# jgsimard/big-dreamer

Measured on AMD Instinct MI355X. Metric: latent transitions/sec (RSSM + imagination) at batch=50 chunk=50 H=15, higher is better.
Workload: dtype f32

## Files before the change

### big_dreamer_amd/_cabi.py

```python
from __future__ import annotations

import ctypes as C
import os

import torch

_HERE = os.path.dirname(os.path.abspath(__file__))
LIB_PATH = os.environ.get("BD_LIB") or os.path.join(_HERE, "libbigdreamer_hip.so")

if not os.path.exists(LIB_PATH):
    raise ImportError(
        f"{LIB_PATH} is missing: the MI355X HIP extension has not been built "
        "(run `python -c 'import __graft_entry__ as g; g.build()'`). There is no CPU fallback.")

lib = C.CDLL(LIB_PATH)

BD_MAX_LAYERS = 6
ACT_NONE, ACT_ELU, ACT_ELU_GRAD = 0, 1, 2
ACT_RELU, ACT_RELU_GRAD, ACT_TANH, ACT_TANH_GRAD = 3, 4, 5, 6
CNN_ACTS = {"ELU": (ACT_ELU, ACT_ELU_GRAD), "ReLU": (ACT_RELU, ACT_RELU_GRAD), "Tanh": (ACT_TANH, ACT_TANH_GRAD)}
GRAD_ACTS = (ACT_ELU_GRAD, ACT_RELU_GRAD, ACT_TANH_GRAD)
P = C.c_void_p
F32 = C.c_float
I32 = C.c_int
# ... 245 lines not shown
    "bd_scan_lds_bytes": (C.c_size_t, [I32] * 8),
    "bd_observe_cluster_set_spin_limit": (I32, [C.c_uint]),
    "bd_observe_cluster_set_ksplit": (I32, [I32]),
    "bd_gauss_head_forward": (I32, [P, P, I32, I32, F32, P, P, P, P]),
    "bd_gauss_head_backward": (I32, [P, P, P, P, P, I32, I32, P, P]),
    "bd_observe_cat_forward": (I32, [C.POINTER(ObserveCatFwdArgs), P]),
    "bd_observe_cat_backward": (I32, [C.POINTER(ObserveCatBwdArgs), P]),
    "bd_observe_cat_cluster_size": (I32, [I32, I32, I32, I32, I32]),
    "bd_observe_cat_cluster_ws_floats": (C.c_size_t, [I32, I32, I32, I32, I32]),
    "bd_observe_cat_forward_cluster": (I32, [C.POINTER(ObserveCatFwdArgs), I32, P, C.c_size_t, P]),
    "bd_observe_cat_backward_cluster": (I32, [C.POINTER(ObserveCatBwdArgs), I32, P, C.c_size_t, P]),
    "bd_imagine_cat_forward": (I32, [C.POINTER(ImagineCatFwdArgs), P]),
    "bd_imagine_cat_backward": (I32, [C.POINTER(ImagineCatBwdArgs), P]),
    "bd_imagine_forward": (I32, [C.POINTER(ImagineFwdArgs), P]),
    "bd_imagine_forward_scan": (I32, [C.POINTER(ImagineFwdArgs), P]),
    "bd_actor_entropy": (I32, [P, P, P, I32, I32, I32, I32, P]),
    "bd_imagine_backward": (I32, [C.POINTER(ImagineBwdArgs), P]),
    "bd_lambda_return_forward": (I32, [P, P, I32, I32, F32, F32, P, P]),
    "bd_rng_fill": (I32, [C.POINTER(RngFillArgs), P]),
    "bd_philox4x32_10": (I32, [C.POINTER(C.c_uint), C.POINTER(C.c_uint), C.POINTER(C.c_uint)]),
    "bd_actor_entropy_rng": (I32, [C.c_ulonglong, C.c_ulonglong, C.c_uint, P, P, I32, I32, I32, I32, P]),
    "bd_gemm_nt": (I32, [P, I32, P, I32, P, I32, I32, I32, I32, I32, P]),
    "bd_categorical_head_forward": (I32, [P, P, I32, I32, I32, P, P, P]),
    "bd_categorical_head_backward": (I32, [P, P, I32, I32, I32, P, P]),
    "bd_kl_categorical_forward": (I32, [P, P, I32, I32, I32, F32, I32, P, I32, P, P]),
    "bd_kl_categorical_backward": (I32, [P, P, I32, I32, I32, F32, F32, F32, F32, P, I32, P, P, P]),
    "bd_plan_rollout": (I32, [C.POINTER(PlanArgs), P]),
    "bd_cem_refit": (I32, [P, I32, P, I32, I32, I32, I32, I32, P, P, P]),
    "bd_plan_rollout_cat": (I32, [C.POINTER(PlanCatArgs), P]),
    "bd_act_step_supported": (I32, [I32, I32, I32, I32, I32, I32]),
    "bd_act_step": (I32, [C.POINTER(ActArgs), P]),
    "bd_act_step_cat_supported": (I32, [I32] * 10),
    "bd_act_step_cat": (I32, [C.POINTER(ActCatArgs), P]),
    "bd_tanh_normal_mode": (I32, [P, P, P, C.c_ulonglong, C.c_ulonglong, C.c_uint, I32, I32, I32, P, P, P]),
    "bd_lambda_return_backward": (I32, [P, F32, I32, I32, F32, F32, P, P, P]),
    "bd_img_heads_supported": (I32, [I32, I32]),
    "bd_img_heads_fwd_bwd": (I32, [C.POINTER(ImgHeadsArgs), P]),
    "bd_actor_reinforce": (I32, [P, P, P, P, P, P, P, I32, I32, I32, F32, F32, F32, I32, P, P, I32, P, P]),
    "bd_actor_reinforce_cat": (I32, [P, P, P, P, P, P, I32, I32, I32, F32, F32, F32, I32, P, P, I32, P, P]),
    "bd_normal_nll": (I32, [P, I32, P, I32, I32, I32, F32, P, I32, P, I32, P, P]),
    "bd_bernoulli_nll": (I32, [P, P, C.c_size_t, F32, P, P, I32, P, P]),
    "bd_kl_forward": (I32, [P, P, P, P, I32, I32, F32, I32, P, I32, P, P]),
    "bd_kl_backward": (I32, [P, P, P, P, I32, I32, F32, F32, F32, F32, P, I32, P, P, P, P, P]),
    "bd_sum": (I32, [P, C.c_size_t, P, I32, P, P]),
    "bd_sumsq": (I32, [P, C.c_size_t, P, I32, P, P]),
    "bd_adam_step": (I32, [P, P, P, P, C.c_size_t, F32, F32, F32, F32, F32, I32, F32, P, I32, P]),
    "bd_polyak": (I32, [P, P, C.c_size_t, F32, P]),
    "bd_replay_gather": (I32, [P, P, I32, I32, P, P]),
    "bd_replay_gather_pixels": (I32, [P, P, I32, I32, I32, P, P, P]),
    "bd_replay_gather_pixels_rng": (I32, [P, P, I32, I32, I32, C.c_ulonglong, C.c_ulonglong, P, P]),
    "bd_replay_append": (I32, [C.POINTER(ReplayAppendArgs), P]),
    "bd_replay_sample_gather": (I32, [C.POINTER(ReplaySampleArgs), P]),
    "bd_reduce_ws_floats": (C.c_size_t, []),
    "bd_conv_gemm": (I32, [C.POINTER(ConvArgs), P]),
    "bd_conv_thin_forward": (I32, [P, I32, I32, I32, I32, I32, P, I32, P, I32, P, P, P]),
    "bd_conv_pack_class": (I32, [P, P, I32, I32, I32, I32, I32, I32, I32, P]),
    "bd_conv_pack_fused": (I32, [P, P, I32, I32, I32, P]),
    "bd_act_backward": (I32, [P, P, C.c_size_t, I32, P]),
    "bd_elu_backward": (I32, [P, P, C.c_size_t, P]),
    "bd_image_layout": (I32, [P, P, I32, I32, I32, I32, P]),
    "bd_eval_frame": (I32, [P, P, I32, U8P, I32, I32, P]),
    "bd_openl_video": (I32, [P, P, I32, I32, U8P, P]),
    "bd_openl_error": (I32, [P, P, I32, I32, I32, I32, P, P]),
    "bd_colsum_ws_floats": (C.c_size_t, [I32]),
    "bd_colsum": (I32, [P, C.c_size_t, I32, P, P, P]),
    "bd_fingerprint": (I32, [C.POINTER(FingerprintArgs), P, P]),
    "bd_diag_ws_floats": (C.c_size_t, []),
    "bd_moments": (I32, [C.POINTER(MomentsArgs), P, P, P]),
    "bd_latent_stats": (I32, [P, P, P, P, I32, I32, P, P, P, P]),
    "bd_latent_stats_categorical": (I32, [P, P, I32, I32, I32, P, P, P, P, P]),
    "bd_segment_sumsq": (I32, [P, I32, C.POINTER(C.c_size_t), P, P, P]),
    "bd_return_range": (I32, [P, I32, I32, I32, C.c_double, C.c_double, P, P, P]),
    "bd_return_seed": (I32, [P, F32, P, C.c_size_t, P, P, I32, P]),
    "bd_actor_reinforce_norm": (I32, [P, P, P, P, P, P, P, P, I32, I32, I32, F32, F32, F32, I32, P, P, I32, P, P]),
    "bd_actor_reinforce_cat_norm": (I32, [P, P, P, P, P, P, P, I32, I32, I32, F32, F32, F32, I32, P, P, I32, P, P]),
    "bd_twohot_decode": (I32, [P, I32, I32, I32, F32, P, P, P]),
    "bd_twohot_decode_backward": (I32, [P, I32, P, I32, I32, F32, P, I32, P]),
    "bd_twohot_nll": (I32, [P, I32, P, P, I32, I32, F32, F32, P, I32, P, P, P]),
}

for _name, (_res, _args) in _SIGS.items():
    _fn = getattr(lib, _name)
    _fn.restype = _res
    _fn.argtypes = _args

EXPORTED = tuple(_SIGS)


def check(rc: int) -> None:
    if rc != 0:
        raise RuntimeError("bigdreamer_hip: " + lib.bd_last_error().decode())


def ptr(t) -> int:
    if t is None:
        return None
    if not (t.dtype in (torch.float32, torch.int64, torch.uint8) and t.is_cuda):
        raise TypeError("expected a CUDA fp32/int64/uint8 tensor")
    if not (t.is_contiguous() or (t.dim() == 2 and t.stride(1) == 1 and t.stride(0) >= t.shape[1])):
        raise ValueError(f"non-contiguous tensor (shape {tuple(t.shape)}, strides {t.stride()}) passed to a HIP kernel: "
                         "call .contiguous() first")
    return t.data_ptr()


def stream() -> int:
    return torch.cuda.current_stream().cuda_stream
# ... 5 lines not shown
```

### big_dreamer_amd/csrc/reduce.hip

```cpp
#include "bd_device.h"
#include "bd_host.h"
#include "bd_discrete.h"
#include "bd_latent.h"

namespace bd {

constexpr int kRedBlocks = 1024;
constexpr float kHalfLog2Pi = 0.91893853320467274178f;

static inline int red_blocks(size_t n) {
    size_t b = (n + 255) / 256;
    return (int)(b < 1 ? 1 : (b > kRedBlocks ? kRedBlocks : b));
}

__global__ __launch_bounds__(256) void final_sum_kernel(const double* __restrict__ partials, int n,
                                                        float* __restrict__ scalars, int slot) {
    __shared__ double red[kWaves];
    double s = 0.0;
    for (int i = threadIdx.x; i < n; i += blockDim.x) s += partials[i];
    s = block_sum_d(s, red);
    if (threadIdx.x == 0) scalars[slot] = (float)s;
}

template <int MODE>
__global__ __launch_bounds__(256) void sum_kernel(const float* __restrict__ x, size_t n, double* __restrict__ partials) {
    __shared__ double red[kWaves];
    double s = 0.0;
    for (size_t i = (size_t)blockIdx.x * blockDim.x + threadIdx.x; i < n; i += (size_t)gridDim.x * blockDim.x) {
        const float v = x[i];
        s += MODE ? (double)v * v : (double)v;
    }
    s = block_sum_d(s, red);
    if (threadIdx.x == 0) partials[blockIdx.x] = s;
}

__global__ __launch_bounds__(256) void normal_nll_kernel(const float* __restrict__ pred, int ldp,
                                                         const float* __restrict__ target, int ldt, int rows, int D,
                                                         float grad_scale, float* __restrict__ dpred, int ldd,
                                                         double* __restrict__ partials) {
    __shared__ double red[kWaves];
    double s = 0.0;
    const size_t n = (size_t)rows * D;
    for (size_t i = (size_t)blockIdx.x * blockDim.x + threadIdx.x; i < n; i += (size_t)gridDim.x * blockDim.x) {
        const size_t r = i / D, c = i - r * D;
        const float d = pred[r * ldp + c] - target[r * ldt + c];
        s += (double)(0.5f * d * d + kHalfLog2Pi);
        if (dpred) dpred[r * ldd + c] = d * grad_scale;
    }
    s = block_sum_d(s, red);
    if (threadIdx.x == 0) partials[blockIdx.x] = s;
}

__global__ __launch_bounds__(256) void bernoulli_nll_kernel(const float* __restrict__ logits, const float* __restrict__ target,
                                                            size_t n, float grad_scale, float* __restrict__ dlogits,
                                                            double* __restrict__ partials) {
    __shared__ double red[kWaves];
    double s = 0.0;
    for (size_t i = (size_t)blockIdx.x * blockDim.x + threadIdx.x; i < n; i += (size_t)gridDim.x * blockDim.x) {
        const float x = logits[i], t = target[i];
        s += (double)(fmaxf(x, 0.f) - x * t + log1pf(expf(-fabsf(x))));
        if (dlogits) dlogits[i] = (1.f / (1.f + expf(-x)) - t) * grad_scale;
    }
    s = block_sum_d(s, red);
    if (threadIdx.x == 0) partials[blockIdx.x] = s;
}

__global__ __launch_bounds__(256) void kl_fwd_kernel(const float* __restrict__ qm, const float* __restrict__ qs,
                                                     const float* __restrict__ pm, const float* __restrict__ ps,
                                                     int rows, int S, float free_nats, int sum_form,
                                                     double* __restrict__ partials) {
    __shared__ double red[kWaves];
    double s = 0.0;
    if (!sum_form) {
        const size_t n = (size_t)rows * S;
        for (size_t i = (size_t)blockIdx.x * blockDim.x + threadIdx.x; i < n; i += (size_t)gridDim.x * blockDim.x)
            s += (double)kl_elem(qm[i], qs[i], pm[i], ps[i]);
    } else {
        for (size_t r = (size_t)blockIdx.x * blockDim.x + threadIdx.x; r < (size_t)rows;
             r += (size_t)gridDim.x * blockDim.x) {
            float rs = 0.f;
            for (int c = 0; c < S; ++c) {
                const size_t i = r * S + c;
                rs += kl_elem(qm[i], qs[i], pm[i], ps[i]);
            }
            s += (double)fmaxf(rs, free_nats);
        }
    }
    s = block_sum_d(s, red);
    if (threadIdx.x == 0) partials[blockIdx.x] = s;
}

__device__ __forceinline__ float max_grad(float x, float fn) { return x < fn ? 0.f : (x == fn ? 0.5f : 1.f); }

__global__ __launch_bounds__(256) void kl_bwd_kernel(const float* __restrict__ qm, const float* __restrict__ qs,
                                                     const float* __restrict__ pm, const float* __restrict__ ps,
                                                     int rows, int S, float free_nats, float kl_balance, float weight,
                                                     float inv_count, const float* __restrict__ scalars, int slot,
                                                     float* __restrict__ dqm, float* __restrict__ dqs,
                                                     float* __restrict__ dpm, float* __restrict__ dps) {
    const size_t n = (size_t)rows * S;
    const bool sum_form = kl_balance == -1.f;
    float fq, fp;
    if (!sum_form) {
        const float f = max_grad(scalars[slot] * inv_count, free_nats) * weight * inv_count;
        fp = kl_balance * f;
        fq = (1.f - kl_balance) * f;
    } else {
        fq = fp = weight / (float)rows;
    }
    for (size_t i = (size_t)blockIdx.x * blockDim.x + threadIdx.x; i < n; i += (size_t)gridDim.x * blockDim.x) {
        float gq = fq, gp = fp;
        if (sum_form) {
            const size_t r = i / S;
            float rs = 0.f;
            for (int c = 0; c < S; ++c) {
                const size_t j = r * S + c;
                rs += kl_elem(qm[j], qs[j], pm[j], ps[j]);
            }
            const float f = max_grad(rs, free_nats);
            gq *= f;
            gp *= f;
        }
        const float a = qm[i], b = qs[i], c = pm[i], d = ps[i];
        const float inv_d = 1.f / d, inv_d2 = inv_d * inv_d, diff = a - c;
        dqm[i] = gq * diff * inv_d2;
        dqs[i] = gq * (b * inv_d2 - 1.f / b);
        dpm[i] = -gp * diff * inv_d2;
        dps[i] = gp * (inv_d - (b * b + diff * diff) * inv_d2 * inv_d);
    }
}

__global__ __launch_bounds__(256) void gauss_head_fwd_kernel(const float* __restrict__ out, const float* __restrict__ eps,
                                                             int M, int S, float min_std, float* __restrict__ mean,
                                                             float* __restrict__ std, float* __restrict__ state) {
    const size_t n = (size_t)M * S;
    for (size_t i = (size_t)blockIdx.x * blockDim.x + threadIdx.x; i < n; i += (size_t)gridDim.x * blockDim.x) {
        const size_t r = i / S, c = i - r * S;
        const float m = out[r * 2 * S + c];
        const float sd = softplusf(out[r * 2 * S + S + c]) + min_std;
        if (mean) mean[i] = m;
        if (std) std[i] = sd;
        if (state) state[i] = m + sd * eps[i];
// ... 5 lines not shown
                                                             const float* __restrict__ dmean,
                                                             const float* __restrict__ dstd, int M, int S,
                                                             float* __restrict__ dout) {
    const size_t n = (size_t)M * S;
    for (size_t i = (size_t)blockIdx.x * blockDim.x + threadIdx.x; i < n; i += (size_t)gridDim.x * blockDim.x) {
        const size_t r = i / S, c = i - r * S;
        const float ds = dstate ? dstate[i] : 0.f;
        const float gm = ds + (dmean ? dmean[i] : 0.f);
        const float gs = (dstate ? ds * eps[i] : 0.f) + (dstd ? dstd[i] : 0.f);
        dout[r * 2 * S + c] = gm;
        dout[r * 2 * S + S + c] = gs * sigmoidf(out[r * 2 * S + S + c]);
    }
}

__global__ __launch_bounds__(256) void lambda_fwd_kernel(const float* __restrict__ reward, const float* __restrict__ value,
                                                         int Hm, int N, float disc, float lam, float* __restrict__ ret) {
    const float one_minus = 1.f - lam, dl = disc * lam;
    for (int n = blockIdx.x * blockDim.x + threadIdx.x; n < N; n += gridDim.x * blockDim.x) {
        const float boot = value[(size_t)(Hm - 1) * N + n];
        float last = boot;
        for (int t = Hm - 1; t >= 0; --t) {
            const float next = (t == Hm - 1) ? boot : value[(size_t)(t + 1) * N + n];
            const float inp = reward[(size_t)t * N + n] + disc * next * one_minus;
            last = inp + dl * last;
            ret[(size_t)t * N + n] = last;
        }
    }
}

__global__ __launch_bounds__(256) void lambda_bwd_kernel(const float* __restrict__ dret, float dconst, int Hm, int N,
                                                         float disc, float lam, float* __restrict__ dreward,
                                                         float* __restrict__ dvalue) {
    const float c = disc * lam, w = disc * (1.f - lam);
    for (int n = blockIdx.x * blockDim.x + threadIdx.x; n < N; n += gridDim.x * blockDim.x) {
        float G = 0.f;
        for (int t = 0; t < Hm; ++t) {
            G = (dret ? dret[(size_t)t * N + n] : dconst) + c * G;
            dreward[(size_t)t * N + n] = G;
            if (t == 0 && Hm > 1) dvalue[n] = 0.f;
            if (t < Hm - 1) {
                dvalue[(size_t)(t + 1) * N + n] = G * w;
            } else {
                const float prev = (Hm > 1) ? dvalue[(size_t)t * N + n] : 0.f;
                dvalue[(size_t)t * N + n] = prev + G * w + c * G;
            }
        }
    }
}

__global__ __launch_bounds__(256) void actor_reinforce_kernel(
    const float* __restrict__ eps, const float* __restrict__ us, const float* __restrict__ stats,
    const float* __restrict__ ret, const float* __restrict__ base0, const float* __restrict__ value,
    const float* __restrict__ weight, const float* __restrict__ ret_scale, int rows, int N, int A, float scale,
    float dentropy, int write, float* __restrict__ dout, double* __restrict__ partials) {
    __shared__ double red[kWaves];
    constexpr float kLn2 = 0.69314718055994531f;
    if (ret_scale) scale /= ret_scale[0];
    double s = 0.0;
    for (int i = blockIdx.x * blockDim.x + threadIdx.x; i < rows; i += gridDim.x * blockDim.x) {
        const float w = weight ? weight[i] : 1.f;
        const float adv = ret[i] - (i < N ? base0[i] : value[i - N]);
        const float c = scale * w * adv;
        const float dent = dentropy * w;
        const float* e = eps + (size_t)i * A;
        const float* uu = us + (size_t)i * 2 * A;
        const float* st = stats + (size_t)i * 4 * A;
        float* d = dout + (size_t)i * 2 * A;
        float l = 0.f;
        for (int j = 0; j < A; ++j) {
            const float ej = e[j], u = uu[j], sd = uu[A + j];
            const float th = st[j], sg = st[A + j];
            const float x = -2.f * u;
            const float sp = fmaxf(x, 0.f) + log1pf(expf(-fabsf(x)));
            l += -0.5f * ej * ej - logf(sd) - kHalfLog2Pi - 2.f * (kLn2 - u - sp);
            const float inv = 1.f / sd, dth = 1.f - th * th;
            float gm = c * (ej * inv) * dth;
            float gr = c * ((ej * ej - 1.f) * inv) * sg;
            if (write) {
                gm += (dent * st[2 * A + j]) * dth;
                gr += (dent * st[3 * A + j]) * sg;
            } else {
                gm += d[j];
                gr += d[A + j];
            }
            d[j] = gm;
            d[A + j] = gr;
        }
        s += (double)(w * l * adv);
    }
    s = block_sum_d(s, red);
    if (threadIdx.x == 0) partials[blockIdx.x] = s;
}

__global__ __launch_bounds__(256) void actor_reinforce_cat_kernel(
    const float* __restrict__ action, const float* __restrict__ stats, const float* __restrict__ ret,
    const float* __restrict__ base0, const float* __restrict__ value, const float* __restrict__ weight,
    const float* __restrict__ ret_scale, int rows, int N, int A, float scale, float dentropy, int write,
    float* __restrict__ dout, double* __restrict__ partials) {
    __shared__ double red[kWaves];
    const int lane = threadIdx.x & 63;
    if (ret_scale) scale /= ret_scale[0];
    const int nw = gridDim.x * (blockDim.x >> 6);
    const bool valid = lane < A;
    double s = 0.0;
    for (int i = blockIdx.x * (blockDim.x >> 6) + (threadIdx.x >> 6); i < rows; i += nw) {
        const float w = weight ? weight[i] : 1.f;
        const float adv = ret[i] - (i < N ? base0[i] : value[i - N]);
        const float c = scale * w * adv;
        const size_t j = (size_t)i * A + lane;
        const float norm = valid ? stats[j] : -INFINITY;
        const unsigned long long hot = __ballot(valid && action[j] > 0.5f);
        const int k = hot ? __builtin_ctzll(hot) : 0;
        const float p = disc_probs(norm, valid);
        const float l = __shfl(norm, k, 64);
        float g = c * ((lane == k ? 1.f : 0.f) - p);
        if (write) {
            const float H = disc_entropy(norm, p, valid);
            g += (dentropy * w) * (-p * (norm + H));
        } else if (valid) {
            g += dout[j];
        }
        if (valid) dout[j] = g;
        if (lane == 0) s += (double)(w * l * adv);
    }
    s = block_sum_d(s, red);
    if (threadIdx.x == 0) partials[blockIdx.x] = s;
}

__global__ __launch_bounds__(256) void adam_kernel(float* __restrict__ p, float* __restrict__ g, float* __restrict__ m,
                                                   float* __restrict__ v, size_t n, float beta1, float beta2, float eps,
                                                   float wd, float step_size, float inv_sqrt_bc2, float max_norm,
                                                   const float* __restrict__ scalars, int sqnorm_slot) {
    const float total_norm = sqrtf(scalars[sqnorm_slot]);
    const float q = max_norm / (total_norm + 1e-6f);
    const float coef = q > 1.f ? 1.f : q;
    for (size_t i = (size_t)blockIdx.x * blockDim.x + threadIdx.x; i < n; i += (size_t)gridDim.x * blockDim.x) {
        const float gc = g[i] * coef;
        g[i] = gc;
        const float pi = p[i];
        const float gw = gc + wd * pi;
        const float mi = m[i] + (1.f - beta1) * (gw - m[i]);
        const float vi = v[i] * beta2 + (1.f - beta2) * gw * gw;
        m[i] = mi;
        v[i] = vi;
        const float denom = sqrtf(vi) * inv_sqrt_bc2 + eps;
        p[i] = pi - step_size * (mi / denom);
    }
}

__global__ __launch_bounds__(256) void polyak_kernel(float* __restrict__ t, const float* __restrict__ s, size_t n, float w) {
    for (size_t i = (size_t)blockIdx.x * blockDim.x + threadIdx.x; i < n; i += (size_t)gridDim.x * blockDim.x)
        t[i] = s[i] * w + t[i] * (1.f - w);
}

__global__ __launch_bounds__(256) void cat_head_fwd_kernel(const float* __restrict__ logits, const float* __restrict__ q,
                                                           size_t groups, int C, float* __restrict__ state,
                                                           float* __restrict__ probs) {
    const int l = threadIdx.x & 31;
    for (size_t g = (size_t)blockIdx.x * 8 + (threadIdx.x >> 5); g < groups; g += (size_t)gridDim.x * 8) {
        const size_t base = g * C;
        float lp[kCatPer];
        group_log_softmax(logits + base, C, l, lp);
        float pr[kCatPer], m = -INFINITY, s = 0.f;
#pragma unroll
        for (int i = 0; i < kCatPer; ++i) m = fmaxf(m, lp[i]);
        m = half_max(m);
#pragma unroll
        for (int i = 0; i < kCatPer; ++i) {
            pr[i] = (l + 32 * i < C) ? expf(lp[i] - m) : 0.f;
            s += pr[i];
        }
        s = half_sum(s);
        float best = -INFINITY;
        int arg = 0x7fffffff;
#pragma unroll
        for (int i = 0; i < kCatPer; ++i) {
            const int c = l + 32 * i;
            if (c < C) {
                pr[i] /= s;
                probs[base + c] = pr[i];
                const float r = pr[i] / q[base + c];
                if (r > best) { best = r; arg = c; }
            }
        }
#pragma unroll
        for (int o = 16; o > 0; o >>= 1) {
            const float ob = __shfl_xor(best, o, 64);
            const int oa = __shfl_xor(arg, o, 64);
            if (ob > best || (ob == best && oa < arg)) { best = ob; arg = oa; }
        }
#pragma unroll
        for (int i = 0; i < kCatPer; ++i) {
            const int c = l + 32 * i;
            if (c < C) state[base + c] = (c == arg) ? 1.f : 0.f;
        }
    }
}

__global__ __launch_bounds__(256) void cat_head_bwd_kernel(const float* __restrict__ dstate, const float* __restrict__ probs,
                                                           size_t groups, int C, float* __restrict__ dlogits) {
    const int l = threadIdx.x & 31;
    for (size_t g = (size_t)blockIdx.x * 8 + (threadIdx.x >> 5); g < groups; g += (size_t)gridDim.x * 8) {
        const size_t base = g * C;
        float pr[kCatPer], gr[kCatPer], dot = 0.f;
#pragma unroll
        for (int i = 0; i < kCatPer; ++i) {
            const int c = l + 32 * i;
            pr[i] = c < C ? probs[base + c] : 0.f;
            gr[i] = c < C ? dstate[base + c] : 0.f;
            dot += pr[i] * gr[i];
        }
        dot = half_sum(dot);
#pragma unroll
        for (int i = 0; i < kCatPer; ++i) {
            const int c = l + 32 * i;
            if (c < C) dlogits[base + c] = pr[i] * (gr[i] - dot);
        }
    }
}

__global__ __launch_bounds__(256) void cat_kl_fwd_kernel(const float* __restrict__ ql, const float* __restrict__ pl, int rows,
                                                         int D, int C, float free_nats, int sum_form,
                                                         double* __restrict__ partials) {
    __shared__ double red[kWaves > 4 ? kWaves : 4];
    const int l = threadIdx.x & 31;
    const size_t units = sum_form ? (size_t)rows : (size_t)rows * D;
    const int per = sum_form ? D : 1;
    double acc = 0.0;
    for (size_t u = (size_t)blockIdx.x * 8 + (threadIdx.x >> 5); u < units; u += (size_t)gridDim.x * 8) {
        float rs = 0.f;
        for (int d = 0; d < per; ++d) {
            const size_t base = (u * per + d) * C;
            float lq[kCatPer], lp[kCatPer];
            group_log_softmax(ql + base, C, l, lq);
            group_log_softmax(pl + base, C, l, lp);
            rs += group_kl(lq, lp, C, l);
        }
        if (l == 0) acc += (double)(sum_form ? fmaxf(rs, free_nats) : rs);
    }
    acc = block_sum_d(acc, red);
    if (threadIdx.x == 0) partials[blockIdx.x] = acc;
}

__global__ __launch_bounds__(256) void cat_kl_bwd_kernel(const float* __restrict__ ql, const float* __restrict__ pl, int rows,
                                                         int D, int C, float free_nats, float kl_balance, float weight,
                                                         float inv_count, const float* __restrict__ scalars, int slot,
                                                         float* __restrict__ dql, float* __restrict__ dpl) {
    const int l = threadIdx.x & 31;
    const bool sum_form = kl_balance == -1.f;
    const size_t units = sum_form ? (size_t)rows : (size_t)rows * D;
    const int per = sum_form ? D : 1;
    float fq, fp;
    if (!sum_form) {
        const float f = max_grad(scalars[slot] * inv_count, free_nats) * weight * inv_count;
        fp = kl_balance * f;
        fq = (1.f - kl_balance) * f;
    } else {
        fq = fp = weight / (float)rows;
    }
    for (size_t u = (size_t)blockIdx.x * 8 + (threadIdx.x >> 5); u < units; u += (size_t)gridDim.x * 8) {
        float f = 1.f;
        if (sum_form) {
            float rs = 0.f;
            for (int d = 0; d < per; ++d) {
                const size_t base = (u * per + d) * C;
                float lq[kCatPer], lp[kCatPer];
                group_log_softmax(ql + base, C, l, lq);
                group_log_softmax(pl + base, C, l, lp);
                rs += group_kl(lq, lp, C, l);
            }
            f = max_grad(rs, free_nats);
        }
        for (int d = 0; d < per; ++d) {
            const size_t base = (u * per + d) * C;
            float lq[kCatPer], lp[kCatPer];
            group_log_softmax(ql + base, C, l, lq);
            group_log_softmax(pl + base, C, l, lp);
            const float kl = group_kl(lq, lp, C, l);
#pragma unroll
            for (int i = 0; i < kCatPer; ++i) {
                const int c = l + 32 * i;
                if (c < C) {
                    const float qv = expf(lq[i]), pv = expf(lp[i]);
                    dql[base + c] = f * fq * (qv == 0.f ? 0.f : qv * (lq[i] - lp[i] - kl));
                    dpl[base + c] = f * fp * (pv - qv);
                }
            }
        }
    }
}

static int finish(double* partials, int nb, float* scalars, int slot, hipStream_t s, const char* name) {
    hipLaunchKernelGGL(final_sum_kernel, dim3(1), dim3(256), 0, s, partials, nb, scalars, slot);
    BD_CHECK_LAUNCH(name);
    return 0;
}

}

extern "C" {
using namespace bd;

size_t bd_reduce_ws_floats(void) { return 2 * (size_t)kRedBlocks; }

int bd_sum(const float* x, size_t n, float* scalars, int slot, float* ws, void* stream) {
    BD_REQUIRE(x && scalars && ws && n > 0, "bd_sum: bad arguments");
    const int nb = red_blocks(n);
    hipLaunchKernelGGL(sum_kernel<0>, dim3(nb), dim3(256), 0, (hipStream_t)stream, x, n, (double*)ws);
    BD_CHECK_LAUNCH("bd_sum");
    return finish((double*)ws, nb, scalars, slot, (hipStream_t)stream, "bd_sum(final)");
}

int bd_actor_reinforce_norm(const float* eps_action, const float* act_us, const float* act_stats, const float* returns,
                            const float* base0, const float* value, const float* weight, const float* ret_scale, int Hm,
                            int N, int A, float rho, float grad_scale, float dentropy, int write, float* d_actor_out,
                            float* scalars, int slot, float* ws, void* stream) {
    BD_REQUIRE(eps_action && act_us && act_stats && returns && base0 && (value || Hm == 1) && d_actor_out && scalars && ws,
               "bd_actor_reinforce: missing pointers");
    BD_REQUIRE(Hm > 0 && N > 0 && A > 0 && (size_t)Hm * N <= (size_t)INT32_MAX / 4 && slot >= 0,
               "bd_actor_reinforce: bad dims (Hm=%d N=%d A=%d slot=%d)", Hm, N, A, slot);
    BD_REQUIRE(rho >= 0.f && rho <= 1.f, "bd_actor_reinforce: gradient mixing %g outside [0, 1]", (double)rho);
    BD_REQUIRE(((size_t)ret_scale & 3u) == 0, "bd_actor_reinforce: ret_scale is not 4-byte aligned");
    const int rows = Hm * N;
    const int nb = red_blocks((size_t)rows);
    hipLaunchKernelGGL(actor_reinforce_kernel, dim3(nb), dim3(256), 0, (hipStream_t)stream, eps_action, act_us, act_stats,
                       returns, base0, value, weight, ret_scale, rows, N, A, -(1.f - rho) * grad_scale, dentropy, write,
                       d_actor_out, (double*)ws);
    BD_CHECK_LAUNCH("bd_actor_reinforce");
    return finish((double*)ws, nb, scalars, slot, (hipStream_t)stream, "bd_actor_reinforce(final)");
}

int bd_actor_reinforce(const float* eps_action, const float* act_us, const float* act_stats, const float* returns,
                       const float* base0, const float* value, const float* weight, int Hm, int N, int A, float rho,
                       float grad_scale, float dentropy, int write, float* d_actor_out, float* scalars, int slot, float* ws,
                       void* stream) {
    return bd_actor_reinforce_norm(eps_action, act_us, act_stats, returns, base0, value, weight, nullptr, Hm, N, A, rho,
                                   grad_scale, dentropy, write, d_actor_out, scalars, slot, ws, stream);
}

int bd_actor_reinforce_cat_norm(const float* action, const float* act_stats, const float* returns, const float* base0,
                                const float* value, const float* weight, const float* ret_scale, int Hm, int N, int A,
                                float rho, float grad_scale, float dentropy, int write, float* d_actor_out, float* scalars,
                                int slot, float* ws, void* stream) {
    BD_REQUIRE(action && act_stats && returns && base0 && (value || Hm == 1) && d_actor_out && scalars && ws,
               "bd_actor_reinforce_cat: missing pointers");
    BD_REQUIRE(Hm > 0 && N > 0 && A > 0 && A <= 64 && (size_t)Hm * N <= (size_t)INT32_MAX / 4 && slot >= 0,
               "bd_actor_reinforce_cat: bad dims (Hm=%d N=%d A=%d slot=%d)", Hm, N, A, slot);
    BD_REQUIRE(rho >= 0.f && rho <= 1.f, "bd_actor_reinforce_cat: gradient mixing %g outside [0, 1]", (double)rho);
    BD_REQUIRE(((size_t)ret_scale & 3u) == 0, "bd_actor_reinforce_cat: ret_scale is not 4-byte aligned");
    const int rows = Hm * N;
    const int nb = red_blocks((size_t)rows);
    hipLaunchKernelGGL(actor_reinforce_cat_kernel, dim3(nb), dim3(256), 0, (hipStream_t)stream, action, act_stats, returns,
                       base0, value, weight, ret_scale, rows, N, A, -(1.f - rho) * grad_scale, dentropy, write, d_actor_out,
                       (double*)ws);
    BD_CHECK_LAUNCH("bd_actor_reinforce_cat");
    return finish((double*)ws, nb, scalars, slot, (hipStream_t)stream, "bd_actor_reinforce_cat(final)");
}

int bd_actor_reinforce_cat(const float* action, const float* act_stats, const float* returns, const float* base0,
                           const float* value, const float* weight, int Hm, int N, int A, float rho, float grad_scale,
                           float dentropy, int write, float* d_actor_out, float* scalars, int slot, float* ws,
                           void* stream) {
    return bd_actor_reinforce_cat_norm(action, act_stats, returns, base0, value, weight, nullptr, Hm, N, A, rho, grad_scale,
                                       dentropy, write, d_actor_out, scalars, slot, ws, stream);
}

int bd_sumsq(const float* x, size_t n, float* scalars, int slot, float* ws, void* stream) {
    BD_REQUIRE(x && scalars && ws && n > 0, "bd_sumsq: bad arguments");
    const int nb = red_blocks(n);
    hipLaunchKernelGGL(sum_kernel<1>, dim3(nb), dim3(256), 0, (hipStream_t)stream, x, n, (double*)ws);
    BD_CHECK_LAUNCH("bd_sumsq");
    return finish((double*)ws, nb, scalars, slot, (hipStream_t)stream, "bd_sumsq(final)");
}

int bd_normal_nll(const float* pred, int ldp, const float* target, int ldt, int rows, int D, float grad_scale,
                  float* dpred, int ldd, float* scalars, int slot, float* ws, void* stream) {
    BD_REQUIRE(pred && target && scalars && ws && rows > 0 && D > 0, "bd_normal_nll: bad arguments");
    BD_REQUIRE(ldp >= D && ldt >= D && (!dpred || ldd >= D), "bd_normal_nll: leading dimension too small");
    const int nb = red_blocks((size_t)rows * D);
    hipLaunchKernelGGL(normal_nll_kernel, dim3(nb), dim3(256), 0, (hipStream_t)stream, pred, ldp, target, ldt, rows, D,
                       grad_scale, dpred, ldd, (double*)ws);
    BD_CHECK_LAUNCH("bd_normal_nll");
    return finish((double*)ws, nb, scalars, slot, (hipStream_t)stream, "bd_normal_nll(final)");
}

int bd_bernoulli_nll(const float* logits, const float* target, size_t n, float grad_scale, float* dlogits, float* scalars,
                     int slot, float* ws, void* stream) {
    BD_REQUIRE(logits && target && scalars && ws && n > 0, "bd_bernoulli_nll: bad arguments");
    const int nb = red_blocks(n);
    hipLaunchKernelGGL(bernoulli_nll_kernel, dim3(nb), dim3(256), 0, (hipStream_t)stream, logits, target, n, grad_scale,
                       dlogits, (double*)ws);
    BD_CHECK_LAUNCH("bd_bernoulli_nll");
    return finish((double*)ws, nb, scalars, slot, (hipStream_t)stream, "bd_bernoulli_nll(final)");
}

int bd_kl_forward(const float* qm, const float* qs, const float* pm, const float* ps, int rows, int S, float free_nats,
                  int sum_form, float* scalars, int slot, float* ws, void* stream) {
    BD_REQUIRE(qm && qs && pm && ps && scalars && ws && rows > 0 && S > 0, "bd_kl_forward: bad arguments");
    const int nb = red_blocks(sum_form ? (size_t)rows : (size_t)rows * S);
    hipLaunchKernelGGL(kl_fwd_kernel, dim3(nb), dim3(256), 0, (hipStream_t)stream, qm, qs, pm, ps, rows, S, free_nats,
                       sum_form, (double*)ws);
    BD_CHECK_LAUNCH("bd_kl_forward");
    return finish((double*)ws, nb, scalars, slot, (hipStream_t)stream, "bd_kl_forward(final)");
}

int bd_kl_backward(const float* qm, const float* qs, const float* pm, const float* ps, int rows, int S, float free_nats,
                   float kl_balance, float weight, float inv_count, const float* scalars, int slot, float* dqm,
                   float* dqs, float* dpm, float* dps, void* stream) {
    BD_REQUIRE(qm && qs && pm && ps && scalars && dqm && dqs && dpm && dps && rows > 0 && S > 0,
               "bd_kl_backward: bad arguments");
    hipLaunchKernelGGL(kl_bwd_kernel, dim3(red_blocks((size_t)rows * S)), dim3(256), 0, (hipStream_t)stream, qm, qs, pm,
                       ps, rows, S, free_nats, kl_balance, weight, inv_count, scalars, slot, dqm, dqs, dpm, dps);
    BD_CHECK_LAUNCH("bd_kl_backward");
    return 0;
}

int bd_gauss_head_forward(const float* out, const float* eps, int M, int S, float min_std, float* mean, float* std,
                          float* state, void* stream) {
    BD_REQUIRE(out && M > 0 && S > 0 && (!state || eps), "bd_gauss_head_forward: bad arguments");
    hipLaunchKernelGGL(gauss_head_fwd_kernel, dim3(red_blocks((size_t)M * S)), dim3(256), 0, (hipStream_t)stream, out, eps,
                       M, S, min_std, mean, std, state);
    BD_CHECK_LAUNCH("bd_gauss_head_forward");
    return 0;
}

int bd_gauss_head_backward(const float* out, const float* eps, const float* dstate, const float* dmean,
                           const float* dstd, int M, int S, float* dout, void* stream) {
    BD_REQUIRE(out && dout && M > 0 && S > 0 && (!dstate || eps), "bd_gauss_head_backward: bad arguments");
    hipLaunchKernelGGL(gauss_head_bwd_kernel, dim3(red_blocks((size_t)M * S)), dim3(256), 0, (hipStream_t)stream, out, eps,
                       dstate, dmean, dstd, M, S, dout);
    BD_CHECK_LAUNCH("bd_gauss_head_backward");
    return 0;
}

int bd_lambda_return_forward(const float* reward, const float* value, int Hm, int N, float discount, float lambda_,
                             float* returns, void* stream) {
    BD_REQUIRE(reward && value && returns && Hm > 0 && N > 0, "bd_lambda_return_forward: bad arguments");
    hipLaunchKernelGGL(lambda_fwd_kernel, dim3(red_blocks(N)), dim3(256), 0, (hipStream_t)stream, reward, value, Hm, N,
                       discount, lambda_, returns);
    BD_CHECK_LAUNCH("bd_lambda_return_forward");
    return 0;
}

int bd_lambda_return_backward(const float* dreturns, float dret_const, int Hm, int N, float discount, float lambda_,
                              float* dreward, float* dvalue, void* stream) {
    BD_REQUIRE(dreward && dvalue && Hm > 0 && N > 0, "bd_lambda_return_backward: bad arguments");
    hipLaunchKernelGGL(lambda_bwd_kernel, dim3(red_blocks(N)), dim3(256), 0, (hipStream_t)stream, dreturns, dret_const, Hm,
                       N, discount, lambda_, dreward, dvalue);
    BD_CHECK_LAUNCH("bd_lambda_return_backward");
    return 0;
}

int bd_adam_step(float* p, float* g, float* m, float* v, size_t n, float lr, float beta1, float beta2, float eps,
                 float weight_decay, int step, float max_norm, const float* scalars, int sqnorm_slot, void* stream) {
    BD_REQUIRE(p && g && m && v && scalars && n > 0 && step >= 1, "bd_adam_step: bad arguments");
    const double bc1 = 1.0 - pow((double)beta1, step), bc2 = 1.0 - pow((double)beta2, step);
    hipLaunchKernelGGL(adam_kernel, dim3(red_blocks(n)), dim3(256), 0, (hipStream_t)stream, p, g, m, v, n, beta1, beta2,
                       eps, weight_decay, (float)(lr / bc1), (float)(1.0 / sqrt(bc2)), max_norm, scalars, sqnorm_slot);
    BD_CHECK_LAUNCH("bd_adam_step");
    return 0;
}

int bd_polyak(float* target, const float* src, size_t n, float weight, void* stream) {
    BD_REQUIRE(target && src && n > 0, "bd_polyak: bad arguments");
    hipLaunchKernelGGL(polyak_kernel, dim3(red_blocks(n)), dim3(256), 0, (hipStream_t)stream, target, src, n, weight);
    BD_CHECK_LAUNCH("bd_polyak");
    return 0;
}

static inline int cat_blocks(size_t units) {
    size_t b = (units + 7) / 8;
    return (int)(b < 1 ? 1 : (b > (size_t)kRedBlocks ? (size_t)kRedBlocks : b));
}

int bd_categorical_head_forward(const float* logits, const float* q_noise, int rows, int D, int C, float* state,
                                float* probs, void* stream) {
    BD_REQUIRE(logits && q_noise && state && probs && rows > 0 && D > 0, "bd_categorical_head_forward: bad arguments");
    BD_REQUIRE(C > 0 && C <= 32 * kCatPer, "bd_categorical_head_forward: %d classes (max %d)", C, 32 * kCatPer);
    const size_t groups = (size_t)rows * D;
    hipLaunchKernelGGL(cat_head_fwd_kernel, dim3(cat_blocks(groups)), dim3(256), 0, (hipStream_t)stream, logits, q_noise,
                       groups, C, state, probs);
    BD_CHECK_LAUNCH("bd_categorical_head_forward");
    return 0;
}

int bd_categorical_head_backward(const float* dstate, const float* probs, int rows, int D, int C, float* dlogits,
                                 void* stream) {
    BD_REQUIRE(dstate && probs && dlogits && rows > 0 && D > 0, "bd_categorical_head_backward: bad arguments");
    BD_REQUIRE(C > 0 && C <= 32 * kCatPer, "bd_categorical_head_backward: %d classes (max %d)", C, 32 * kCatPer);
    const size_t groups = (size_t)rows * D;
    hipLaunchKernelGGL(cat_head_bwd_kernel, dim3(cat_blocks(groups)), dim3(256), 0, (hipStream_t)stream, dstate, probs,
                       groups, C, dlogits);
    BD_CHECK_LAUNCH("bd_categorical_head_backward");
    return 0;
}

int bd_kl_categorical_forward(const float* post_logits, const float* prior_logits, int rows, int D, int C, float free_nats,
                              int sum_form, float* scalars, int slot, float* ws, void* stream) {
    BD_REQUIRE(post_logits && prior_logits && scalars && ws && rows > 0 && D > 0, "bd_kl_categorical_forward: bad arguments");
    BD_REQUIRE(C > 0 && C <= 32 * kCatPer, "bd_kl_categorical_forward: %d classes (max %d)", C, 32 * kCatPer);
    const int nb = cat_blocks(sum_form ? (size_t)rows : (size_t)rows * D);
    hipLaunchKernelGGL(cat_kl_fwd_kernel, dim3(nb), dim3(256), 0, (hipStream_t)stream, post_logits, prior_logits, rows, D, C,
                       free_nats, sum_form, (double*)ws);
    BD_CHECK_LAUNCH("bd_kl_categorical_forward");
    return finish((double*)ws, nb, scalars, slot, (hipStream_t)stream, "bd_kl_categorical_forward(final)");
}

int bd_kl_categorical_backward(const float* post_logits, const float* prior_logits, int rows, int D, int C, float free_nats,
                               float kl_balance, float weight, float inv_count, const float* scalars, int slot,
                               float* dpost, float* dprior, void* stream) {
    BD_REQUIRE(post_logits && prior_logits && scalars && dpost && dprior && rows > 0 && D > 0,
               "bd_kl_categorical_backward: bad arguments");
    BD_REQUIRE(C > 0 && C <= 32 * kCatPer, "bd_kl_categorical_backward: %d classes (max %d)", C, 32 * kCatPer);
    const bool sum_form = kl_balance == -1.f;
    hipLaunchKernelGGL(cat_kl_bwd_kernel, dim3(cat_blocks(sum_form ? (size_t)rows : (size_t)rows * D)), dim3(256), 0,
                       (hipStream_t)stream, post_logits, prior_logits, rows, D, C, free_nats, kl_balance, weight, inv_count,
                       scalars, slot, dpost, dprior);
    BD_CHECK_LAUNCH("bd_kl_categorical_backward");
    return 0;
}

}
```

### include/bigdreamer_hip.h

```cpp
#ifndef BIGDREAMER_HIP_H
#define BIGDREAMER_HIP_H

#include <stddef.h>
#include <stdint.h>

#ifdef __cplusplus
extern "C" {
#endif

#define BD_MAX_LAYERS 6
#define BD_ACT_NONE 0
#define BD_ACT_ELU 1
#define BD_ACT_ELU_GRAD 2
#define BD_ACT_RELU 3
#define BD_ACT_RELU_GRAD 4
#define BD_ACT_TANH 5
#define BD_ACT_TANH_GRAD 6

const char* bd_last_error(void);
int bd_version(void);

#define BD_PACK_COPY 0
#define BD_PACK_PRODUCT 1
#define BD_PACK_PRODUCT_VEC 2
// ... 521 lines not shown
int bd_replay_gather(const float* src, const int64_t* idx, int n_idx, int width, float* dst, void* stream);

int bd_replay_gather_pixels(const unsigned char* src, const int64_t* idx, int n_idx, int pixels, int bit_depth,
                            const float* noise, float* dst, void* stream);
int bd_replay_gather_pixels_rng(const unsigned char* src, const int64_t* idx, int n_idx, int pixels, int bit_depth,
                                unsigned long long seed, unsigned long long step, float* dst, void* stream);

typedef struct {
    int n;
    int size;
    const int32_t* rows;
    const float* obs;
    int obs_width;
    int bit_depth;
    void* dst_obs;
    const float* act;
    int A;
    float* dst_act;
    const float* reward;
    const float* nonterminal;
    float* dst_reward;
    float* dst_nonterminal;
} bd_replay_append_args;
int bd_replay_append(const bd_replay_append_args* a, void* stream);

typedef struct {
    const void* obs;
    const float* act;
    const float* reward;
    const float* nonterminal;
    int obs_width;
    int A;
    int size;
    int lanes;
    int lane_size;
    int idx;
    int full;
    int n;
    int L;
    int bit_depth;
    unsigned long long seed;
    unsigned long long step;
    unsigned long long pix_seed;
    unsigned long long pix_step;
    float* dst_obs;
    float* dst_act;
    float* dst_reward;
    float* dst_nonterminal;
    int64_t* idx_out;
} bd_replay_sample_args;
int bd_replay_sample_gather(const bd_replay_sample_args* a, void* stream);

size_t bd_reduce_ws_floats(void);

#define BD_FP_MAX_BUFFERS 16
typedef struct {
    int n_buf;
    struct {
        const float* p;
        size_t n;
    } buf[BD_FP_MAX_BUFFERS];
} bd_fingerprint_args;
int bd_fingerprint(const bd_fingerprint_args* a, unsigned long long* out, void* stream);

size_t bd_diag_ws_floats(void);

#define BD_MOMENTS_MAX_BUFFERS 16
#define BD_MOMENTS_WORDS 6
typedef struct {
    int n_buf;
    struct {
        const float* p;
        const float* q;
        size_t n;
    } buf[BD_MOMENTS_MAX_BUFFERS];
} bd_moments_args;
int bd_moments(const bd_moments_args* a, double* out, float* ws, void* stream);

#define BD_LATENT_WORDS 15
int bd_latent_stats(const float* qm, const float* qs, const float* pm, const float* ps, int rows, int S, double* out,
                    double* colsum, float* ws, void* stream);

#define BD_LATENT_CAT_WORDS 5
int bd_latent_stats_categorical(const float* post_logits, const float* prior_logits, int rows, int D, int C, double* out,
                                double* colsum, unsigned* used, float* ws, void* stream);

#define BD_SEGMENTS_MAX 32
int bd_segment_sumsq(const float* x, int n_seg, const size_t* offsets, double* out, float* ws, void* stream);

int bd_return_range(const float* returns, int M, int k_lo, int k_hi, double decay, double floor_, double* state,
                    float* range, void* stream);
int bd_return_seed(const float* range, float dret_const, const float* weight, size_t n, float* dreturns, float* scalars,
                   int slot, void* stream);

int bd_twohot_decode(const float* logits, int ld, int rows, int K, float zmax, float* value, float* mean, void* stream);
int bd_twohot_decode_backward(const float* logits, int ld, const float* dvalue, int rows, int K, float zmax, float* dlogits,
                              int ldd, void* stream);
int bd_twohot_nll(const float* logits, int ld, const float* target, const float* weight, int rows, int K, float zmax,
                  float grad_scale, float* dlogits, int ldd, float* value, float* row_loss, void* stream);

#ifdef __cplusplus
}
#endif
#endif
```

Before: 13.99 million.

## Finish scalar reductions in-kernel via last-block atomic counter instead of second launch

```diff
diff --git a/big_dreamer_amd/_cabi.py b/big_dreamer_amd/_cabi.py
--- a/big_dreamer_amd/_cabi.py
+++ b/big_dreamer_amd/_cabi.py
@@ -321,6 +321,7 @@
     "bd_replay_append": (I32, [C.POINTER(ReplayAppendArgs), P]),
     "bd_replay_sample_gather": (I32, [C.POINTER(ReplaySampleArgs), P]),
     "bd_reduce_ws_floats": (C.c_size_t, []),
+    "bd_reduce_set_finish": (I32, [I32]),
     "bd_conv_gemm": (I32, [C.POINTER(ConvArgs), P]),
     "bd_conv_thin_forward": (I32, [P, I32, I32, I32, I32, I32, P, I32, P, I32, P, P, P]),
     "bd_conv_pack_class": (I32, [P, P, I32, I32, I32, I32, I32, I32, I32, P]),
diff --git a/big_dreamer_amd/csrc/reduce.hip b/big_dreamer_amd/csrc/reduce.hip
--- a/big_dreamer_amd/csrc/reduce.hip
+++ b/big_dreamer_amd/csrc/reduce.hip
@@ -1,9 +1,73 @@
+#include <atomic>
+#include <mutex>
+
 #include "bd_device.h"
 #include "bd_host.h"
 #include "bd_discrete.h"
 #include "bd_latent.h"
 
 namespace bd {
+
+constexpr int kFinishSets = 64;
+constexpr int kFinishShards = 32;
+constexpr int kFinishFlat = 64;
+static_assert(kFinishShards <= kFinishFlat, "the top word of a sharded grid counts kFinishShards arrivals");
+struct alignas(128) FinishWord {
+    unsigned v;
+    unsigned pad[31];
+};
+__device__ FinishWord finish_words[kFinishSets][1 + kFinishShards];
+
+struct Finish {
+    int set;
+    int slot;
+    float* scalars;
+};
+
+typedef __attribute__((address_space(1))) unsigned gu32;
+typedef __attribute__((address_space(1))) unsigned long long gu64;
+
+__device__ __forceinline__ void finish_block(double s, double* __restrict__ partials, const Finish& fin, double* red) {
+    const int nb = (int)gridDim.x, b = (int)blockIdx.x;
+    if (fin.set < 0) {
+        if (threadIdx.x == 0) partials[b] = s;
+        return;
+    }
+    __shared__ int last;
+    gu64* gp = (gu64*)(unsigned long long*)partials;
+    if (threadIdx.x == 0) {
+        __hip_atomic_store(gp + b, (unsigned long long)__double_as_longlong(s), __ATOMIC_RELAXED, __HIP_MEMORY_SCOPE_AGENT);
+        asm volatile("s_waitcnt vmcnt(0)" ::: "memory");
+        gu32* top = (gu32*)&finish_words[fin.set][0].v;
+        bool l;
+        if (nb <= kFinishFlat) {
+            l = __hip_atomic_fetch_add(top, 1u, __ATOMIC_RELAXED, __HIP_MEMORY_SCOPE_AGENT) == (unsigned)(nb - 1);
+        } else {
+            const int sh = b % kFinishShards;
+            const unsigned pop = (unsigned)((nb - sh + kFinishShards - 1) / kFinishShards);
+            gu32* sw = (gu32*)&finish_words[fin.set][1 + sh].v;
+            l = __hip_atomic_fetch_add(sw, 1u, __ATOMIC_RELAXED, __HIP_MEMORY_SCOPE_AGENT) == pop - 1;
+            if (l) {
+                __hip_atomic_store(sw, 0u, __ATOMIC_RELAXED, __HIP_MEMORY_SCOPE_AGENT);
+                l = __hip_atomic_fetch_add(top, 1u, __ATOMIC_RELAXED, __HIP_MEMORY_SCOPE_AGENT) ==
+                    (unsigned)(kFinishShards - 1);
+            }
+        }
+        if (l) {
+            __hip_atomic_store(top, 0u, __ATOMIC_RELAXED, __HIP_MEMORY_SCOPE_AGENT);
+            __builtin_amdgcn_fence(__ATOMIC_ACQUIRE, "agent");
+            asm volatile("s_waitcnt vmcnt(0)" ::: "memory");
+        }
+        last = l;
+    }
+    __syncthreads();
+    if (!last) return;
+    double t = 0.0;
+    for (int i = threadIdx.x; i < nb; i += blockDim.x)
+        t += __longlong_as_double((long long)__hip_atomic_load(gp + i, __ATOMIC_RELAXED, __HIP_MEMORY_SCOPE_AGENT));
+    t = block_sum_d(t, red);
+    if (threadIdx.x == 0) fin.scalars[fin.slot] = (float)t;
+}
 
 constexpr int kRedBlocks = 1024;
 constexpr float kHalfLog2Pi = 0.91893853320467274178f;
@@ -23,7 +87,7 @@
 }
 
 template <int MODE>
-__global__ __launch_bounds__(256) void sum_kernel(const float* __restrict__ x, size_t n, double* __restrict__ partials) {
+__global__ __launch_bounds__(256) void sum_kernel(const float* __restrict__ x, size_t n, double* __restrict__ partials, Finish fin) {
     __shared__ double red[kWaves];
     double s = 0.0;
     for (size_t i = (size_t)blockIdx.x * blockDim.x + threadIdx.x; i < n; i += (size_t)gridDim.x * blockDim.x) {
@@ -31,13 +95,13 @@
         s += MODE ? (double)v * v : (double)v;
     }
     s = block_sum_d(s, red);
-    if (threadIdx.x == 0) partials[blockIdx.x] = s;
+    finish_block(s, partials, fin, red);
 }
 
 __global__ __launch_bounds__(256) void normal_nll_kernel(const float* __restrict__ pred, int ldp,
                                                          const float* __restrict__ target, int ldt, int rows, int D,
                                                          float grad_scale, float* __restrict__ dpred, int ldd,
-                                                         double* __restrict__ partials) {
+                                                         double* __restrict__ partials, Finish fin) {
     __shared__ double red[kWaves];
     double s = 0.0;
     const size_t n = (size_t)rows * D;
@@ -48,12 +112,12 @@
         if (dpred) dpred[r * ldd + c] = d * grad_scale;
     }
     s = block_sum_d(s, red);
-    if (threadIdx.x == 0) partials[blockIdx.x] = s;
+    finish_block(s, partials, fin, red);
 }
 
 __global__ __launch_bounds__(256) void bernoulli_nll_kernel(const float* __restrict__ logits, const float* __restrict__ target,
                                                             size_t n, float grad_scale, float* __restrict__ dlogits,
-                                                            double* __restrict__ partials) {
+                                                            double* __restrict__ partials, Finish fin) {
     __shared__ double red[kWaves];
     double s = 0.0;
     for (size_t i = (size_t)blockIdx.x * blockDim.x + threadIdx.x; i < n; i += (size_t)gridDim.x * blockDim.x) {
@@ -62,13 +126,13 @@
         if (dlogits) dlogits[i] = (1.f / (1.f + expf(-x)) - t) * grad_scale;
     }
     s = block_sum_d(s, red);
-    if (threadIdx.x == 0) partials[blockIdx.x] = s;
+    finish_block(s, partials, fin, red);
 }
 
 __global__ __launch_bounds__(256) void kl_fwd_kernel(const float* __restrict__ qm, const float* __restrict__ qs,
                                                      const float* __restrict__ pm, const float* __restrict__ ps,
                                                      int rows, int S, float free_nats, int sum_form,
-                                                     double* __restrict__ partials) {
+                                                     double* __restrict__ partials, Finish fin) {
     __shared__ double red[kWaves];
     double s = 0.0;
     if (!sum_form) {
@@ -87,7 +151,7 @@
         }
     }
     s = block_sum_d(s, red);
-    if (threadIdx.x == 0) partials[blockIdx.x] = s;
+    finish_block(s, partials, fin, red);
 }
 
 __device__ __forceinline__ float max_grad(float x, float fn) { return x < fn ? 0.f : (x == fn ? 0.5f : 1.f); }
@@ -199,7 +263,7 @@
     const float* __restrict__ eps, const float* __restrict__ us, const float* __restrict__ stats,
     const float* __restrict__ ret, const float* __restrict__ base0, const float* __restrict__ value,
     const float* __restrict__ weight, const float* __restrict__ ret_scale, int rows, int N, int A, float scale,
-    float dentropy, int write, float* __restrict__ dout, double* __restrict__ partials) {
+    float dentropy, int write, float* __restrict__ dout, double* __restrict__ partials, Finish fin) {
     __shared__ double red[kWaves];
     constexpr float kLn2 = 0.69314718055994531f;
     if (ret_scale) scale /= ret_scale[0];
@@ -236,14 +300,14 @@
         s += (double)(w * l * adv);
     }
     s = block_sum_d(s, red);
-    if (threadIdx.x == 0) partials[blockIdx.x] = s;
+    finish_block(s, partials, fin, red);
 }
 
 __global__ __launch_bounds__(256) void actor_reinforce_cat_kernel(
     const float* __restrict__ action, const float* __restrict__ stats, const float* __restrict__ ret,
     const float* __restrict__ base0, const float* __restrict__ value, const float* __restrict__ weight,
     const float* __restrict__ ret_scale, int rows, int N, int A, float scale, float dentropy, int write,
-    float* __restrict__ dout, double* __restrict__ partials) {
+    float* __restrict__ dout, double* __restrict__ partials, Finish fin) {
     __shared__ double red[kWaves];
     const int lane = threadIdx.x & 63;
     if (ret_scale) scale /= ret_scale[0];
@@ -271,7 +335,7 @@
         if (lane == 0) s += (double)(w * l * adv);
     }
     s = block_sum_d(s, red);
-    if (threadIdx.x == 0) partials[blockIdx.x] = s;
+    finish_block(s, partials, fin, red);
 }
 
 __global__ __launch_bounds__(256) void adam_kernel(float* __restrict__ p, float* __restrict__ g, float* __restrict__ m,
@@ -368,7 +432,7 @@
 
 __global__ __launch_bounds__(256) void cat_kl_fwd_kernel(const float* __restrict__ ql, const float* __restrict__ pl, int rows,
                                                          int D, int C, float free_nats, int sum_form,
-                                                         double* __restrict__ partials) {
+                                                         double* __restrict__ partials, Finish fin) {
     __shared__ double red[kWaves > 4 ? kWaves : 4];
     const int l = threadIdx.x & 31;
     const size_t units = sum_form ? (size_t)rows : (size_t)rows * D;
@@ -386,7 +450,7 @@
         if (l == 0) acc += (double)(sum_form ? fmaxf(rs, free_nats) : rs);
     }
     acc = block_sum_d(acc, red);
-    if (threadIdx.x == 0) partials[blockIdx.x] = acc;
+    finish_block(acc, partials, fin, red);
 }
 
 __global__ __launch_bounds__(256) void cat_kl_bwd_kernel(const float* __restrict__ ql, const float* __restrict__ pl, int rows,
@@ -437,7 +501,25 @@
     }
 }
 
-static int finish(double* partials, int nb, float* scalars, int slot, hipStream_t s, const char* name) {
+static std::atomic<int> finish_mode{1};
+static std::mutex finish_mu;
+static const void* finish_ws[kFinishSets];
+static int finish_known = 0;
+
+static int finish_index(const void* ws) {
+    if (!finish_mode.load(std::memory_order_relaxed)) return -1;
+    std::lock_guard<std::mutex> lock(finish_mu);
+    for (int i = 0; i < finish_known; ++i)
+        if (finish_ws[i] == ws) return i;
+    if (finish_known == kFinishSets) return -1;
+    finish_ws[finish_known] = ws;
+    return finish_known++;
+}
+
+static inline Finish finish_arg(const float* ws, float* scalars, int slot) { return Finish{finish_index(ws), slot, scalars}; }
+
+static int finish(const Finish& fin, double* partials, int nb, float* scalars, int slot, hipStream_t s, const char* name) {
+    if (fin.set >= 0) return 0;
     hipLaunchKernelGGL(final_sum_kernel, dim3(1), dim3(256), 0, s, partials, nb, scalars, slot);
     BD_CHECK_LAUNCH(name);
     return 0;
@@ -449,13 +531,22 @@
 using namespace bd;
 
 size_t bd_reduce_ws_floats(void) { return 2 * (size_t)kRedBlocks; }
+
+int bd_reduce_set_finish(int mode) {
+    BD_REQUIRE(mode == 0 || mode == 1, "bd_reduce_set_finish: mode %d (0: two launches, 1: in-kernel)", mode);
+    std::lock_guard<std::mutex> lock(bd::finish_mu);
+    bd::finish_mode.store(mode, std::memory_order_relaxed);
+    bd::finish_known = 0;
+    return 0;
+}
 
 int bd_sum(const float* x, size_t n, float* scalars, int slot, float* ws, void* stream) {
     BD_REQUIRE(x && scalars && ws && n > 0, "bd_sum: bad arguments");
     const int nb = red_blocks(n);
-    hipLaunchKernelGGL(sum_kernel<0>, dim3(nb), dim3(256), 0, (hipStream_t)stream, x, n, (double*)ws);
+    const Finish fin = finish_arg(ws, scalars, slot);
+    hipLaunchKernelGGL(sum_kernel<0>, dim3(nb), dim3(256), 0, (hipStream_t)stream, x, n, (double*)ws, fin);
     BD_CHECK_LAUNCH("bd_sum");
-    return finish((double*)ws, nb, scalars, slot, (hipStream_t)stream, "bd_sum(final)");
+    return finish(fin, (double*)ws, nb, scalars, slot, (hipStream_t)stream, "bd_sum(final)");
 }
 
 int bd_actor_reinforce_norm(const float* eps_action, const float* act_us, const float* act_stats, const float* returns,
@@ -470,11 +561,12 @@
     BD_REQUIRE(((size_t)ret_scale & 3u) == 0, "bd_actor_reinforce: ret_scale is not 4-byte aligned");
     const int rows = Hm * N;
     const int nb = red_blocks((size_t)rows);
+    const Finish fin = finish_arg(ws, scalars, slot);
     hipLaunchKernelGGL(actor_reinforce_kernel, dim3(nb), dim3(256), 0, (hipStream_t)stream, eps_action, act_us, act_stats,
                        returns, base0, value, weight, ret_scale, rows, N, A, -(1.f - rho) * grad_scale, dentropy, write,
-                       d_actor_out, (double*)ws);
+                       d_actor_out, (double*)ws, fin);
     BD_CHECK_LAUNCH("bd_actor_reinforce");
-    return finish((double*)ws, nb, scalars, slot, (hipStream_t)stream, "bd_actor_reinforce(final)");
+    return finish(fin, (double*)ws, nb, scalars, slot, (hipStream_t)stream, "bd_actor_reinforce(final)");
 }
 
 int bd_actor_reinforce(const float* eps_action, const float* act_us, const float* act_stats, const float* returns,
@@ -497,11 +589,12 @@
     BD_REQUIRE(((size_t)ret_scale & 3u) == 0, "bd_actor_reinforce_cat: ret_scale is not 4-byte aligned");
     const int rows = Hm * N;
     const int nb = red_blocks((size_t)rows);
+    const Finish fin = finish_arg(ws, scalars, slot);
     hipLaunchKernelGGL(actor_reinforce_cat_kernel, dim3(nb), dim3(256), 0, (hipStream_t)stream, action, act_stats, returns,
                        base0, value, weight, ret_scale, rows, N, A, -(1.f - rho) * grad_scale, dentropy, write, d_actor_out,
-                       (double*)ws);
+                       (double*)ws, fin);
     BD_CHECK_LAUNCH("bd_actor_reinforce_cat");
-    return finish((double*)ws, nb, scalars, slot, (hipStream_t)stream, "bd_actor_reinforce_cat(final)");
+    return finish(fin, (double*)ws, nb, scalars, slot, (hipStream_t)stream, "bd_actor_reinforce_cat(final)");
 }
 
 int bd_actor_reinforce_cat(const float* action, const float* act_stats, const float* returns, const float* base0,
@@ -515,9 +608,10 @@
 int bd_sumsq(const float* x, size_t n, float* scalars, int slot, float* ws, void* stream) {
     BD_REQUIRE(x && scalars && ws && n > 0, "bd_sumsq: bad arguments");
     const int nb = red_blocks(n);
-    hipLaunchKernelGGL(sum_kernel<1>, dim3(nb), dim3(256), 0, (hipStream_t)stream, x, n, (double*)ws);
+    const Finish fin = finish_arg(ws, scalars, slot);
+    hipLaunchKernelGGL(sum_kernel<1>, dim3(nb), dim3(256), 0, (hipStream_t)stream, x, n, (double*)ws, fin);
     BD_CHECK_LAUNCH("bd_sumsq");
-    return finish((double*)ws, nb, scalars, slot, (hipStream_t)stream, "bd_sumsq(final)");
+    return finish(fin, (double*)ws, nb, scalars, slot, (hipStream_t)stream, "bd_sumsq(final)");
 }
 
 int bd_normal_nll(const float* pred, int ldp, const float* target, int ldt, int rows, int D, float grad_scale,
@@ -525,30 +619,33 @@
     BD_REQUIRE(pred && target && scalars && ws && rows > 0 && D > 0, "bd_normal_nll: bad arguments");
     BD_REQUIRE(ldp >= D && ldt >= D && (!dpred || ldd >= D), "bd_normal_nll: leading dimension too small");
     const int nb = red_blocks((size_t)rows * D);
+    const Finish fin = finish_arg(ws, scalars, slot);
     hipLaunchKernelGGL(normal_nll_kernel, dim3(nb), dim3(256), 0, (hipStream_t)stream, pred, ldp, target, ldt, rows, D,
-                       grad_scale, dpred, ldd, (double*)ws);
+                       grad_scale, dpred, ldd, (double*)ws, fin);
     BD_CHECK_LAUNCH("bd_normal_nll");
-    return finish((double*)ws, nb, scalars, slot, (hipStream_t)stream, "bd_normal_nll(final)");
+    return finish(fin, (double*)ws, nb, scalars, slot, (hipStream_t)stream, "bd_normal_nll(final)");
 }
 
 int bd_bernoulli_nll(const float* logits, const float* target, size_t n, float grad_scale, float* dlogits, float* scalars,
                      int slot, float* ws, void* stream) {
     BD_REQUIRE(logits && target && scalars && ws && n > 0, "bd_bernoulli_nll: bad arguments");
     const int nb = red_blocks(n);
+    const Finish fin = finish_arg(ws, scalars, slot);
     hipLaunchKernelGGL(bernoulli_nll_kernel, dim3(nb), dim3(256), 0, (hipStream_t)stream, logits, target, n, grad_scale,
-                       dlogits, (double*)ws);
+                       dlogits, (double*)ws, fin);
     BD_CHECK_LAUNCH("bd_bernoulli_nll");
-    return finish((double*)ws, nb, scalars, slot, (hipStream_t)stream, "bd_bernoulli_nll(final)");
+    return finish(fin, (double*)ws, nb, scalars, slot, (hipStream_t)stream, "bd_bernoulli_nll(final)");
 }
 
 int bd_kl_forward(const float* qm, const float* qs, const float* pm, const float* ps, int rows, int S, float free_nats,
                   int sum_form, float* scalars, int slot, float* ws, void* stream) {
     BD_REQUIRE(qm && qs && pm && ps && scalars && ws && rows > 0 && S > 0, "bd_kl_forward: bad arguments");
     const int nb = red_blocks(sum_form ? (size_t)rows : (size_t)rows * S);
+    const Finish fin = finish_arg(ws, scalars, slot);
     hipLaunchKernelGGL(kl_fwd_kernel, dim3(nb), dim3(256), 0, (hipStream_t)stream, qm, qs, pm, ps, rows, S, free_nats,
-                       sum_form, (double*)ws);
+                       sum_form, (double*)ws, fin);
     BD_CHECK_LAUNCH("bd_kl_forward");
-    return finish((double*)ws, nb, scalars, slot, (hipStream_t)stream, "bd_kl_forward(final)");
+    return finish(fin, (double*)ws, nb, scalars, slot, (hipStream_t)stream, "bd_kl_forward(final)");
 }
 
 int bd_kl_backward(const float* qm, const float* qs, const float* pm, const float* ps, int rows, int S, float free_nats,
@@ -647,10 +744,11 @@
     BD_REQUIRE(post_logits && prior_logits && scalars && ws && rows > 0 && D > 0, "bd_kl_categorical_forward: bad arguments");
     BD_REQUIRE(C > 0 && C <= 32 * kCatPer, "bd_kl_categorical_forward: %d classes (max %d)", C, 32 * kCatPer);
     const int nb = cat_blocks(sum_form ? (size_t)rows : (size_t)rows * D);
+    const Finish fin = finish_arg(ws, scalars, slot);
     hipLaunchKernelGGL(cat_kl_fwd_kernel, dim3(nb), dim3(256), 0, (hipStream_t)stream, post_logits, prior_logits, rows, D, C,
-                       free_nats, sum_form, (double*)ws);
+                       free_nats, sum_form, (double*)ws, fin);
     BD_CHECK_LAUNCH("bd_kl_categorical_forward");
-    return finish((double*)ws, nb, scalars, slot, (hipStream_t)stream, "bd_kl_categorical_forward(final)");
+    return finish(fin, (double*)ws, nb, scalars, slot, (hipStream_t)stream, "bd_kl_categorical_forward(final)");
 }
 
 int bd_kl_categorical_backward(const float* post_logits, const float* prior_logits, int rows, int D, int C, float free_nats,
diff --git a/include/bigdreamer_hip.h b/include/bigdreamer_hip.h
--- a/include/bigdreamer_hip.h
+++ b/include/bigdreamer_hip.h
@@ -597,6 +597,7 @@
 int bd_replay_sample_gather(const bd_replay_sample_args* a, void* stream);
 
 size_t bd_reduce_ws_floats(void);
+int bd_reduce_set_finish(int mode);
 
 #define BD_FP_MAX_BUFFERS 16
 typedef struct {
```

Result: no change. 13.94 million (-0.3%).
